# SLebailly/Ignis-MasterThesis

Measured on AMD Instinct MI355X. Metric: Mrays/s (primary+secondary) at fixed spp; per-pixel L2 vs CPU ref, higher is better.
Workload: dtype f32; 1 GPU; diamond_scene.json 1000x1000, 256 spp = 32 iterations x spi 8, path tracer max_depth 64, seed 0; scene=diamond_scene.json, width=1000, height=1000, spp=256, spi=8, parallelism=single GPU

## Files before the change

### ignis-masterthesis_amd/csrc/igx_device.hip

```cpp
#include "igx.h"

#include "device_math.h"
#include "device_scene.h"
#include "igx_kernels.h"
#include "../host/bvh_build.h"
#include "../host/light_select.h"

#include <hip/hip_runtime.h>

#include <algorithm>
#include <array>
#include <chrono>
#include <map>
#include <cmath>
#include <cstring>
#include <condition_variable>
#include <deque>
#include <memory>
#include <mutex>
#include <string>
#include <thread>
#include <vector>
#include <type_traits>

using namespace igxd;

#ifndef IGX_PART
#define IGX_PART 0
#endif

namespace igxh {

constexpr int BLOCK = 256;
[[maybe_unused]] constexpr int MAX_BLOCKS_PER_CU = 8;
[[maybe_unused]] constexpr int MAX_STACK = 128;
constexpr int MAX_BOUNCES = 256;
constexpr long long MAX_CHUNK_PATHS = 1ll << 27;
constexpr int SLOT_BITS = 27;
constexpr uint32_t SLOT_MASK = (1u << SLOT_BITS) - 1;
[[maybe_unused]] constexpr int MAX_ENCLOSING = 31;
static_assert(MAX_CHUNK_PATHS <= (1ll << SLOT_BITS), "path slots must fit the slot bits");
#ifndef EXTEND_WAVES
#define EXTEND_WAVES 4
#endif
#ifndef EXTEND_WAVES_FULL
#define EXTEND_WAVES_FULL 3
#endif
#ifndef EXTEND_WAVES_LDS
// ... 108 lines not shown
}

static_assert(NSH == 64 && BLOCK % 64 == 0 && NSH % WAVES_PER_BLOCK == 0, "one shard counter per lane of a wave");
static_assert(BLOCK == TSTACK_STRIDE, "traversal stacks are laid out for BLOCK threads");

__device__ __forceinline__ int row_total(const int* row) {
    const int* r = row + lane_id() * CSTRIDE;
    int v = r[0] + r[1] + r[2];
    for (int off = 32; off > 0; off >>= 1) v += __shfl_xor(v, off);
    return __builtin_amdgcn_readfirstlane(v);
}

struct WaveWork {
    int s, k, K;
};
__device__ __forceinline__ WaveWork wave_work() {
    const int g = __builtin_amdgcn_readfirstlane((int)blockIdx.x * WAVES_PER_BLOCK + (int)(threadIdx.x >> 6));
    return WaveWork{g % NSH, g / NSH, (int)gridDim.x * WAVES_PER_BLOCK / NSH};
}

__device__ __forceinline__ int gen_index(int i, int shard_cap) {
    return ((i >> 6) & (NSH - 1)) * shard_cap + ((i >> 12) << 6) + (i & 63);
}
__device__ __forceinline__ int gen_shard_count(int n, int s) {
    const int rem = (n & (64 * NSH - 1)) - s * 64;
    return (n >> 12) * 64 + (rem < 0 ? 0 : (rem > 64 ? 64 : rem));
}

struct ShardCount {
    int a, ab, n;
};
__device__ __forceinline__ ShardCount shard_count(const int* cnt, int s) {
    const int a = uniform_load(cnt + s * CSTRIDE), b = uniform_load(cnt + s * CSTRIDE + 1);
// ... 495 lines not shown
    const GenPath g = gen_path(fa, sv, i);
    PathState ps;
    ps.o = g.o;
    ps.d = g.d;
    ps.counter = g.counter;
    ps.seed = g.seed;
    ps.depth = g.depth;
    ps.slot = i;
    ps.contrib = mk(1, 1, 1);
    ps.inv_pdf = 0;
    ps.eta = 1.0f;
    ps.inside = -1;
    return ps;
}

template <int V0, bool STATS, bool LDS>
__global__ void __launch_bounds__(BLOCK, LDS ? EXTEND_WAVES_LDS : (variant_full(V0) ? EXTEND_WAVES_FULL : EXTEND_WAVES)) k_extend(FrameArgs fa, SceneView gsv, PathBuf in, PathBuf out, ShadowBuf sh,
                                                  float4* L, KernelCounters kc, int tail_threshold) {
    constexpr int V = LDS ? kernel_variant(V0, true) : (EXTEND_TREELET ? kernel_variant(V0, false) : V0);
    __shared__ int stack_mem[LDS_STACK * BLOCK];
    extern __shared__ float4 lds_scene[];
    const TStack ts = make_tstack(stack_mem, LDS_STACK, gsv.spill);
    const bool gen = fa.gen_n > 0;
    if (!gen && row_total(kc.cnt_in) <= tail_threshold) return;
    const SceneView sv = LDS ? stage_scene_lds<BLOCK>(gsv, lds_scene) : stage_treelet<BLOCK>(gsv, lds_scene);
    TraceStats st{0, 0, 0, 0, 0, 0, 0};
    __shared__ unsigned long long cls_mem[STATS ? WAVES_PER_BLOCK * 36 : 1];
    if constexpr (STATS) {
        st.cls = cls_mem + 36 * (threadIdx.x >> 6);
        if (lane_id() < 36) st.cls[lane_id()] = 0;
    }
    const WaveWork w = wave_work();
    int s = w.s;
    auto count_of = [&](int sh_) {
        if (gen) {
            const int g = gen_shard_count(fa.gen_n, sh_);
            return ShardCount{g, g, g};
        }
        return shard_count(kc.cnt_in, sh_);
    };
    ShardCount sc = count_of(s);
    uint64_t done = 0;
    int p0 = w.k * 64;
    int claimed = -1;
    unsigned long long t_last = STATS ? __builtin_amdgcn_s_memtime() : 0;
    for (;;) {
        if (fa.dynamic) {
// ... 724 lines not shown
    int stream_slots = 2;
    int concurrent_opt = 1;
    int concurrent_start_pct = 10;
    int tail_pairs_opt = -1;
    int64_t treelet_opt = -1;
    bool tree_dirty = true;
    int tree_ext = 0, tree_shadow = 0;
    int64_t tail_opt = -1;
    int64_t tail_last_opt = -1;
    bool fuse_generate = true;
    int split_opt = -1;
    int refill_opt = -1;
    int shadow_ifif_opt = -1;
    int64_t lds_scene_max = 48 * 1024;
    size_t lds_scene_bytes = 0;
    size_t table_bytes = 0;
    size_t shading_bytes = 0;
    int leaf_size = 4;
    int classify_opt = 4;
    int shadow_classes_opt = 1;
    int dynamic_opt = DYN_EXTEND | DYN_REFILL_TRACE | DYN_REFILL_SHADOW;
    int group_order_opt = -1;
    int face_normals_opt = 1;
    int face_shade_opt = 1;
    float sah_node_cost = 1.0f;
    int bvh_bins = 32;
    int bvh_bins_tlas = 32;
    bool spatial_splits = false;
    bool rebuild_bvh = false;
    bool has_scene = false;
// ... 146 lines not shown
    s.pa.shard_cap = s.pb.shard_cap = s.sh.shard_cap = shard_cap;
    s.cap = cap;
    s.shard_cap = shard_cap;
    return IGX_OK;
}

hipEvent_t slot_event(Slot& s) {
    if (s.ev_next >= s.ev_pool.size()) {
        hipEvent_t e;
        (void)hipEventCreate(&e);
        s.ev_pool.push_back(e);
    }
    return s.ev_pool[s.ev_next++];
}

int grid_for(igx_device* dev, long long items, int blocks_per_cu) {
    const long long q = GRID_QUANTUM;
    long long need = (items + BLOCK - 1) / BLOCK;
    long long cap = (long long)dev->num_cus * std::min(blocks_per_cu, MAX_BLOCKS_PER_CU);
    long long g = std::min((need + q - 1) / q * q, std::max(q, cap / q * q));
    return (int)std::max(q, g);
}

#endif

constexpr size_t SPLIT_TABLE_BYTES = 64u << 20;
#ifndef GROUP_ORDER_AUTO
#define GROUP_ORDER_AUTO 0
#endif
inline bool use_tail_pairs(const igx_device* dev) {
    return dev->lds_scene_bytes == 0 && (dev->tail_pairs_opt < 0 ? true : dev->tail_pairs_opt != 0);
}
inline size_t tree_bytes(const igx_device* dev, int nodes) { return (size_t)nodes * dev->nf4 * 16; }
inline int refill_min(const igx_device* dev) { return dev->refill_opt >= 0 ? dev->refill_opt : 16; }
// ... 25 lines not shown
        case 1: MACRO(1); break;              \
        case 2: MACRO(2); break;              \
        case 3: MACRO(3); break;              \
        case 4: MACRO(4); break;              \
        case 5: MACRO(5); break;              \
        case 6: MACRO(6); break;              \
        case 7: MACRO(7); break;              \
        case 2 | VARIANT_Q4: MACRO(130); break; \
        case 3 | VARIANT_Q4: MACRO(131); break; \
        case 6 | VARIANT_Q4: MACRO(134); break; \
        default: MACRO(135); break;           \
        }                                     \
    } while (0)

template <bool STATS>
void launch_extend(igx_device* dev, Slot& s, int grid, const FrameArgs& fa, const PathBuf& in, const PathBuf& out,
                   const KernelCounters& kc, int tail) {
    if (dev->lds_scene_bytes) {
#define L_EXTL(S) hipLaunchKernelGGL((k_extend<S, STATS, true>), dim3(grid), dim3(BLOCK), dev->lds_scene_bytes, dev->stream, fa, dev->sv, in, out, s.sh, s.L, kc, tail)
        IGX_DISPATCH_VARIANT8(dev->variant, L_EXTL);
#undef L_EXTL
        return;
    }
    SceneView tsv = dev->sv;
    tsv.tree_n = dev->tree_ext;
#define L_EXT(S) hipLaunchKernelGGL((k_extend<S, STATS, false>), dim3(grid), dim3(BLOCK), tree_bytes(dev, tsv.tree_n), dev->stream, fa, tsv, in, out, s.sh, s.L, kc, tail)
    IGX_DISPATCH_VARIANT8(dev->variant, L_EXT);
#undef L_EXT
}
template <bool STATS>
void launch_trace(igx_device* dev, Slot& s, int grid, const FrameArgs& fa, const PathBuf& in, const int* cnt, int tail,
                  int* work) {
// ... 62 lines not shown
#undef L_FINL
        return;
    }
    if (use_tail_pairs(dev)) {
#define L_FINP(S) hipLaunchKernelGGL((k_finish_pairs<S, STATS>), dim3(grid), dim3(BLOCK), tree_bytes(dev, tsv.tree_n), dev->tail_stream, fa, tsv, in, s.L, cnt, tail, dev->dstats, dev->tail_counts)
        IGX_DISPATCH_VARIANT8(dev->variant, L_FINP);
#undef L_FINP
        return;
    }
#define L_FIN(S) hipLaunchKernelGGL((k_finish<S, STATS, false>), dim3(grid), dim3(BLOCK), tree_bytes(dev, tsv.tree_n), dev->tail_stream, fa, tsv, in, s.L, cnt, tail, dev->dstats, dev->tail_counts)
    IGX_DISPATCH_VARIANT8(dev->variant, L_FIN);
#undef L_FIN
}

template <typename K>
int resident_blocks(K kernel, size_t dyn_lds = 0) {
    int nb = 0;
    if (hipOccupancyMaxActiveBlocksPerMultiprocessor(&nb, kernel, BLOCK, dyn_lds) != hipSuccess || nb < 1) nb = 1;
    return nb;
}
#define IGX_RES1(K, V, ...) return lds ? resident_blocks(K<V, __VA_ARGS__, true>, lds) : resident_blocks(K<V, __VA_ARGS__, false>, tree)
#define IGX_RESIDENT(K, ...)                                         \
    do {                                                             \
        switch (v & (3 | VARIANT_Q4)) {                              \
        case 0: IGX_RES1(K, 0, __VA_ARGS__);                         \
        case 1: IGX_RES1(K, 1, __VA_ARGS__);                         \
        case 2: IGX_RES1(K, 2, __VA_ARGS__);                         \
        case 3: IGX_RES1(K, 3, __VA_ARGS__);                         \
        case 2 | VARIANT_Q4: IGX_RES1(K, 130, __VA_ARGS__);          \
        default: IGX_RES1(K, 131, __VA_ARGS__);                      \
        }                                                            \
    } while (0)
#define IGX_RESIDENT8(K, ...)                                        \
    do {                                                             \
// ... 52 lines not shown
int shade_blocks_per_cu(bool full) { return full ? resident_blocks(k_shade<true>) : resident_blocks(k_shade<false>); }
#endif

#define IGX_EXTEND_HELPERS(X, S)                                                                                     \
    X void launch_extend<S>(igx_device*, Slot&, int, const FrameArgs&, const PathBuf&, const PathBuf&,               \
                            const KernelCounters&, int);                                                             \
    X int extend_blocks_per_cu<S>(int, size_t, size_t);
#define IGX_FINISH_HELPERS(X, S)                                                                                     \
    X void launch_finish<S>(igx_device*, Slot&, int, const FrameArgs&, const PathBuf&, const int*, int);             \
    X int finish_blocks_per_cu<S>(int, size_t, size_t, bool);
#define IGX_TRACE_HELPERS(X, S)                                                                                      \
    X void launch_trace<S>(igx_device*, Slot&, int, const FrameArgs&, const PathBuf&, const int*, int, int*);              \
    X void launch_shadow<S>(igx_device*, Slot&, int, const int*, int*, hipStream_t);                                       \
    X int trace_blocks_per_cu<S>(int, size_t, bool);                                                                  \
    X int shadow_blocks_per_cu<S>(int, size_t, bool, size_t);
#if IGX_PART == 1
IGX_EXTEND_HELPERS(template, true)
IGX_EXTEND_HELPERS(template, false)
#else
IGX_EXTEND_HELPERS(extern template, true)
IGX_EXTEND_HELPERS(extern template, false)
#endif
#if IGX_PART == 2
IGX_FINISH_HELPERS(template, true)
IGX_FINISH_HELPERS(template, false)
#else
IGX_FINISH_HELPERS(extern template, true)
IGX_FINISH_HELPERS(extern template, false)
#endif
#if IGX_PART == 3
// ... 43 lines not shown
    if ((st = ::wait_idle(dev)) || (st = harvest(dev, dev->slots[0])) || (st = harvest(dev, dev->slots[1]))) return st;
    HIPCHK(hipStreamSynchronize(dev->stream));
    HIPCHK(hipStreamSynchronize(dev->stream2));
    HIPCHK(hipStreamSynchronize(dev->shadow_stream));
    HIPCHK(hipStreamSynchronize(dev->tail_stream));
    unsigned long long tc[2] = {0, 0};
    HIPCHK(hipMemcpy(tc, dev->tail_counts, sizeof(tc), hipMemcpyDeviceToHost));
    HIPCHK(hipMemset(dev->tail_counts, 0, sizeof(tc)));
    dev->stats.bounce_rays += tc[0];
    dev->stats.shadow_rays += tc[1];
    dev->stats.tail_bounce_rays += tc[0];
    dev->stats.tail_shadow_rays += tc[1];
    return IGX_OK;
}

void configure_treelet(igx_device* dev) {
    dev->tree_ext = dev->tree_shadow = 0;
    dev->tree_dirty = false;
    if (!dev->has_scene || dev->lds_scene_bytes || dev->treelet_opt == 0) return;
    int cap = (int)std::min<size_t>(TREELET_FRONT, (size_t)dev->sv.num_nodes);
    if (dev->treelet_opt > 0) cap = (int)std::min<int64_t>(cap, dev->treelet_opt);
    const int v = dev->variant;
    const bool refill = use_refill(dev);
    auto fit = [&](auto blocks) {
        const int nb0 = blocks((size_t)0);
        int lo = 0, hi = cap;
        while (lo < hi) {
            const int mid = (lo + hi + 1) / 2;
            if (blocks(tree_bytes(dev, mid)) >= nb0) lo = mid;
            else hi = mid - 1;
// ... 63 lines not shown
extern "C" igx_status igx_create(int hip_device, igx_device** out) {
    if (!out) return IGX_ERR_INVALID_ARGUMENT;
    *out = nullptr;
    igx_device* dev = new igx_device();
    dev->hip_device = hip_device;
    hipError_t e = hipSetDevice(hip_device);
    if (e != hipSuccess) {
        delete dev;
        return IGX_ERR_HIP;
    }
    hipDeviceProp_t prop;
    if (hipGetDeviceProperties(&prop, hip_device) == hipSuccess) {
        dev->num_cus = prop.multiProcessorCount;
        dev->mem_total = prop.totalGlobalMem;
    }
    if (hipStreamCreateWithFlags(&dev->stream, hipStreamNonBlocking) != hipSuccess ||
        hipStreamCreateWithFlags(&dev->stream2, hipStreamNonBlocking) != hipSuccess ||
        hipStreamCreateWithFlags(&dev->tail_stream, hipStreamNonBlocking) != hipSuccess ||
        hipStreamCreateWithFlags(&dev->shadow_stream, hipStreamNonBlocking) != hipSuccess) {
        delete dev;
        return IGX_ERR_HIP;
    }
    if (hipMalloc((void**)&dev->dstats, DSTATS * sizeof(unsigned long long)) != hipSuccess ||
        hipMalloc((void**)&dev->tail_counts, 2 * sizeof(unsigned long long)) != hipSuccess) {
        delete dev;
        return IGX_ERR_OUT_OF_MEMORY;
    }
    (void)hipMemset(dev->dstats, 0, DSTATS * sizeof(unsigned long long));
    (void)hipMemset(dev->tail_counts, 0, 2 * sizeof(unsigned long long));
    *out = dev;
// ... 84 lines not shown
    else if (k == "fuse_generate") dev->fuse_generate = value != 0;
    else if (k == "split") {
        if (value < -1 || value > 1) return fail(dev, IGX_ERR_INVALID_ARGUMENT, "split must be -1 (auto), 0 or 1");
        dev->split_opt = (int)value;
    }
    else if (k == "shadow_ifif") {
        if (value < -1 || value > 1) return fail(dev, IGX_ERR_INVALID_ARGUMENT, "shadow_ifif must be -1 (auto), 0 or 1");
        dev->shadow_ifif_opt = (int)value;
    }
    else if (k == "refill") {
        if (value < -1 || value > 64) return fail(dev, IGX_ERR_INVALID_ARGUMENT, "refill must be -1 (auto) or in [0, 64]");
        dev->refill_opt = (int)value;
    }
    else if (k == "lds_scene_max") {
        dev->lds_scene_max = value;
        size_t b = ((size_t)dev->sv.num_nodes * dev->sv.node_f4 + (size_t)dev->sv.num_inst * 4 +
                    (size_t)dev->sv.num_tris * 3) * 16;
        dev->lds_scene_bytes = dev->has_scene && (int64_t)b <= value ? b : 0;
    }
    else if (k == "full_shading") dev->full_shading_opt = value != 0;
    else if (k == "enclosing") dev->enclosing_opt = value != 0;
    else if (k == "bvh_width") {
        if (value != 0 && value != 2 && value != 4) return fail(dev, IGX_ERR_INVALID_ARGUMENT, "bvh_width must be 0 (auto), 2 or 4");
        dev->bvh_width_opt = (int)value;
    }
    else if (k == "spatial_splits") dev->spatial_splits = value != 0;
    else if (k == "rebuild_bvh") dev->rebuild_bvh = value != 0;
    else if (k == "dynamic") dev->dynamic_opt = (int)(value & 15);
    else if (k == "group_order") {
        if (value < -1 || value > 1) return fail(dev, IGX_ERR_INVALID_ARGUMENT, "group_order must be -1 (auto), 0 (A, B, C) or 1 (C, B, A)");
        dev->group_order_opt = (int)value;
    }
    else if (k == "face_normals") dev->face_normals_opt = value != 0;
// ... 628 lines not shown
    }
    if (fn_tab.empty()) sv.fn_tab = nullptr;
    if (fsh.empty()) sv.fsh = nullptr;
    if (uvs.empty()) sv.uv = nullptr;
    sv.tlas_root = tlas_root;
    sv.num_nodes = (int)(nodes.size() / nf4);
    sv.node_f4 = nf4;
    dev->bvh_width = width;
    dev->quantized = quantize;
    dev->nf4 = nf4;
    sv.num_inst = (int)(inst.size() / 4);
    sv.num_enc = (int)enc_tab.size();
    sv.num_tris = (int)(tris.size() / 3);
    {
        size_t b = ((size_t)sv.num_nodes * nf4 + (size_t)sv.num_inst * 4 + (size_t)sv.num_tris * 3) * 16;
        const size_t bl = b;
        dev->lds_scene_bytes = (int64_t)bl <= dev->lds_scene_max ? bl : 0;
        dev->table_bytes = b;
        dev->shading_bytes = ent.size() * sizeof(ent[0]) + vtx.size() * sizeof(vtx[0]) + nrm.size() * sizeof(nrm[0]) +
                             idx.size() * sizeof(idx[0]) + mats.size() * sizeof(DevMaterial) + lights.size() * sizeof(lights[0]) +
                             fn_tab.size() * sizeof(fn_tab[0]) + fsh.size() * sizeof(fsh[0]);
    }
    sv.num_lights = (int)lights.size();
    sv.num_infinite = num_infinite;
    sv.selector = lsel.selector;
    float dx = desc->scene_bbox_max[0] - desc->scene_bbox_min[0];
    float dy = desc->scene_bbox_max[1] - desc->scene_bbox_min[1];
    float dz = desc->scene_bbox_max[2] - desc->scene_bbox_min[2];
    sv.scene_radius = std::sqrt(dx * dx + dy * dy + dz * dz) / 2 * 1.01f;
    if (desc->technique.max_depth > 255) {
        free_scene(dev);
        return fail(dev, IGX_ERR_UNSUPPORTED, "max_depth above 255 is not supported (8-bit path depth)");
    }
// ... 24 lines not shown
    if (textured) dev->full_shading = true;
    if (dev->aov_on) dev->full_shading = true;
    for (uint32_t e = 0; textured && e < desc->num_entities; ++e) {
        const igx_entity& en = desc->entities[e];
        if (desc->materials[en.material].texture != IGX_TEXTURE_NONE && desc->shapes[en.shape].type == IGX_SHAPE_SPHERE) {
            free_scene(dev);
            return fail(dev, IGX_ERR_UNSUPPORTED, "textured material on an analytic sphere (texture coordinates of spheres are not supported)");
        }
    }
    if ((st = configure_stack(dev)) != IGX_OK) {
        free_scene(dev);
        return st;
    }
    dev->has_scene = true;
    dev->tree_dirty = true;
    return IGX_OK;
}

struct ChunkPlan {
    FrameArgs fa{};
    DevCamera cam{};
    int iteration = 0, spi = 1, count = 1, width = 1;
    long long local_pixels = 0, chunk_pixels_max = 0;
    int iters_per_chunk = 1;
    size_t slot_cap = 0;
    int max_bounces = 1, ext_bpc = 1, sh_bpc = 1, fin_bpc = 1;
    bool pairs = false;
};
struct SchedItem {
    bool clear = false;
// ... 134 lines not shown
            r.fa.chunk_iters = std::min(pl.iters_per_chunk, pl.count - r.it0);
            r.chunk_pixels = (int)std::min<long long>(pl.chunk_pixels_max, pl.local_pixels - r.px0);
            r.fa.chunk_pixel0 = (int)r.px0;
            r.fa.chunk_pixels = r.chunk_pixels;
            r.n = (long long)r.chunk_pixels * pl.spi * r.fa.chunk_iters;
            r.live = r.n;
            const long long fin_lanes = (long long)pl.fin_bpc * dev->num_cus * BLOCK / (pl.pairs ? 2 : 1);
            const int64_t topt = r.last_of_plan && dev->tail_last_opt >= 0 ? dev->tail_last_opt : dev->tail_opt;
            r.tail = topt >= 0 ? (int)std::min<int64_t>(topt, 1 << 30) : (int)std::max<long long>(32768, std::min(r.n / 64, fin_lanes));
            S.tail = r.tail;
            S.camera = valid_pixels_in_chunk(r.fa) * pl.spi * r.fa.chunk_iters;
            S.n0 = r.n;
            S.split = false;
            S.bounce_ev.clear();
            S.launched = 0;
            r.ext_grid = grid_for(dev, r.n, pl.ext_bpc);
            r.sh_grid = grid_for(dev, r.n, pl.sh_bpc);
            r.fin_grid = grid_for(dev, std::min<long long>(r.n, r.tail) * (pl.pairs ? 2 : 1), pl.fin_bpc);
            r.fuse_gen = dev->fuse_generate && r.n > r.tail;
            use_slot(r);
            IGX_CC(hipMemsetAsync(S.ctr, 0, (size_t)(2 * pl.max_bounces + 4) * CROW * sizeof(int), dev->stream));
            if (dev->dynamic_opt)
                IGX_CC(hipMemsetAsync(S.ctr + (size_t)WORK_ROW0 * CROW, 0, (size_t)4 * pl.max_bounces * CROW * sizeof(int), dev->stream));
            if (!r.fuse_gen) {
                begin_timed(S, 2, -1, dev->stream);
                hipLaunchKernelGGL(k_generate, dim3(grid_for(dev, r.n, 8)), dim3(BLOCK), 0, dev->stream, r.fa, dev->sv, S.pa, S.L, S.ctr);
                end_timed(S, dev->stream);
                IGX_CC(hipGetLastError());
            }
            restore();
            if (r.n <= r.tail) {
// ... 19 lines not shown
                    IGX_CC(q);
                    r.live = row_total(S, 2 * (r.b - 1));
                    if (r.live <= r.tail) {
                        r.switch_b = r.b - 1;
                        r.loop_done = true;
                        break;
                    }
                }
                const int b = r.b;
                PathBuf in = (b & 1) ? S.pb : S.pa, out = (b & 1) ? S.pa : S.pb;
                KernelCounters kc{row(2 * b), row(2 * (b + 1)), row(2 * b + 1), dev->dstats, row(WORK_ROW0 + 4 * b)};
                begin_timed(S, 0, b, dev->stream);
                FrameArgs fb = r.fa;
                fb.gen_n = r.fuse_gen && b == 0 ? (int)r.n : 0;
                const long long bound = IGX_LIVE_GRID && b >= 2 ? r.live : r.n;
                const int ext_grid = IGX_LIVE_GRID ? grid_for(dev, bound, pl.ext_bpc) : r.ext_grid;
                const int sh_grid = IGX_LIVE_GRID ? grid_for(dev, bound, pl.sh_bpc) : r.sh_grid;
                if (inst) launch_extend<true>(dev, S, ext_grid, fb, in, out, kc, r.tail);
                else launch_extend<false>(dev, S, ext_grid, fb, in, out, kc, r.tail);
                end_timed(S, dev->stream);
                begin_timed(S, 1, b, dev->stream);
                int* const sh_work =
                    (dev->dynamic_opt & (use_refill(dev) ? DYN_REFILL_SHADOW : DYN_SHADOW)) ? row(WORK_ROW0 + 4 * b + 2) : nullptr;
                if (inst) launch_shadow<true>(dev, S, sh_grid, row(2 * b + 1), sh_work, dev->stream);
                else launch_shadow<false>(dev, S, sh_grid, row(2 * b + 1), sh_work, dev->stream);
                end_timed(S, dev->stream);
                IGX_CC(hipGetLastError());
                IGX_CC(hipMemcpyAsync(S.pinned + (size_t)(2 * b + 1) * CROW, row(2 * b + 1), 2 * CROW * sizeof(int),
                                      hipMemcpyDeviceToHost, dev->stream));
                hipEvent_t e = slot_event(S);
                IGX_CC(hipEventRecord(e, dev->stream));
// ... 295 lines not shown
    if (dev->slot_budget_mb > 0)
        auto_chunk_paths = std::max<long long>(1ll << 20, std::min<long long>(auto_chunk_paths, slot_budget / (dev->stream_slots * path_slot_bytes)));
    long long cap = dev->capacity_opt > 0 ? dev->capacity_opt
                                          : (count > 1 ? auto_chunk_paths : std::min<long long>({total_paths, 1ll << 24, auto_chunk_paths}));
    cap = std::min<long long>(cap, MAX_CHUNK_PATHS);
    cap = std::max<long long>(p->spi, (cap / p->spi) * p->spi);
    const long long chunk_pixels_max = std::min<long long>(cap, total_paths) / p->spi;
    const int iters_per_chunk = total_paths <= cap ? (int)std::min<long long>(count, cap / total_paths) : 1;
    const size_t slot_cap = (size_t)(chunk_pixels_max * p->spi * iters_per_chunk);

    const int max_bounces = std::min(std::max(dev->sv.max_depth, 1), MAX_BOUNCES - 1);
    const bool inst = dev->instrument;
    const int sd = dev->variant;
    const size_t ldsb = dev->lds_scene_bytes;
    if (dev->tree_dirty) configure_treelet(dev);
    const int ext_bpc = inst ? extend_blocks_per_cu<true>(sd, ldsb, tree_bytes(dev, dev->tree_ext))
                             : extend_blocks_per_cu<false>(sd, ldsb, tree_bytes(dev, dev->tree_ext));
    const bool refill = use_refill(dev);
    const int tr_bpc = inst ? trace_blocks_per_cu<true>(sd, dev->lds_scene_bytes, refill)
                            : trace_blocks_per_cu<false>(sd, dev->lds_scene_bytes, refill);
    const bool full = variant_full(sd);
    const int shade_bpc = shade_blocks_per_cu(full);
    const int sh_bpc = inst ? shadow_blocks_per_cu<true>(sd, dev->lds_scene_bytes, refill, tree_bytes(dev, dev->tree_shadow))
                            : shadow_blocks_per_cu<false>(sd, dev->lds_scene_bytes, refill, tree_bytes(dev, dev->tree_shadow));
    const bool pairs = use_tail_pairs(dev);
    const int fin_bpc = inst ? finish_blocks_per_cu<true>(sd, ldsb, 0, pairs) : finish_blocks_per_cu<false>(sd, ldsb, 0, pairs);

    if (conc) {
        auto plan = std::make_shared<ChunkPlan>();
        plan->fa = fa;
        plan->cam = cam;
        plan->iteration = p->iteration;
// ... 79 lines not shown
        const bool overlap = split && dev->overlap_shadow_opt;
        hipStream_t sh_strm = overlap ? dev->shadow_stream : dev->stream;
        hipEvent_t sh_done = nullptr;
        if (n <= tail) switch_b = 0;
        for (int b = 0; switch_b < 0 && b < max_bounces; ++b) {
            long long bound = n;
            if (b >= 2) {
                HIPCHK(hipEventSynchronize(S.bounce_ev[b - 2]));
                bound = row_total(S, 2 * (b - 1));
                if (bound <= tail) {
                    switch_b = b - 1;
                    break;
                }
            }
            if (!IGX_LIVE_GRID) bound = n;
            const int ext_grid = grid_for(dev, bound, ext_bpc), tr_grid = grid_for(dev, bound, tr_bpc);
            const int shade_grid = grid_for(dev, bound, shade_bpc), sh_grid = grid_for(dev, bound, sh_bpc);
            PathBuf in = (b & 1) ? S.pb : S.pa, out = (b & 1) ? S.pa : S.pb;
            KernelCounters kc{row(2 * b), row(2 * (b + 1)), row(2 * b + 1), dev->dstats, row(WORK_ROW0 + 4 * b)};
            if (split) {
                begin_timed(5, b, dev->stream);
                int* const tr_work = (dev->dynamic_opt & DYN_REFILL_TRACE) ? row(WORK_ROW0 + 4 * b) : nullptr;
                if (inst) launch_trace<true>(dev, S, tr_grid, fa, in, row(2 * b), tail, tr_work);
                else launch_trace<false>(dev, S, tr_grid, fa, in, row(2 * b), tail, tr_work);
                end_timed(dev->stream);
                if (sh_done) HIPCHK(hipStreamWaitEvent(dev->stream, sh_done, 0));
                begin_timed(0, b, dev->stream);
                launch_shade(dev, full, shade_grid, fa, in, S.hb, out, S.sh, S.L, kc, tail);
                end_timed(dev->stream);
            } else {
                begin_timed(0, b, dev->stream);
// ... 224 lines not shown
    out->leaf_visits = h[1];
    out->tri_tests = h[2];
    out->blas_enters = h[3];
    out->shadow_node_visits = h[4];
    out->shadow_leaf_visits = h[5];
    out->shadow_tri_tests = h[6];
    out->shadow_blas_enters = h[7];
    out->shaded_hits = h[8];
    out->wave_node_iters = h[9];
    out->wave_leaf_iters = h[10];
    out->shadow_wave_node_iters = h[11];
    out->shadow_wave_leaf_iters = h[12];
    out->bvh_width = dev->bvh_width;
    out->node_bytes = dev->nf4 * 16;
    out->lds_scene_bytes = (int32_t)dev->lds_scene_bytes;
    if (dev->has_scene && dev->tree_dirty) configure_treelet(dev);
    out->shadow_blocks_per_cu = dev->has_scene ? shadow_blocks_per_cu<false>(dev->variant, dev->lds_scene_bytes, use_refill(dev),
                                                                            tree_bytes(dev, dev->tree_shadow)) : 0;
    out->treelet_nodes[0] = dev->tree_ext;
    out->treelet_nodes[1] = 0;
    out->treelet_nodes[2] = dev->tree_shadow;
    out->treelet_nodes[3] = 0;
    out->table_bytes = dev->table_bytes;
    out->shading_bytes = dev->shading_bytes;
    out->slot_bytes = 0;
    for (const Slot& s : dev->slots)
        out->slot_bytes += (uint64_t)s.shard_cap * NSH * (2 * 56 * (s.pa.c_base ? 2 : 1) + 48 + (s.hb.h ? 20 : 0)) +
                           (uint64_t)s.cap * (16 + (s.aov_di ? 32 : 0));
    return IGX_OK;
}
// ... 62 lines not shown
```

### ignis-masterthesis_amd/csrc/igx_kernels.h

```cpp
#pragma once

#include "device_math.h"
#include "device_scene.h"

namespace igxd {

struct SceneView {
    const float4* nodes;
    const float4* tris;
    const float4* inst;
    const float4* spheres;
    const float4* ent;
    const float4* vtx;
    const float4* nrm;
    const int4* idx;
    const DevMaterial* mats;
    const DevLight* lights;
    int tlas_root;
    int num_lights;
    int num_infinite;
    float scene_radius;
    DevCamera cam;
    int max_depth, min_depth, nee;
    float clamp;
// ... 1 lines not shown
    const float4* tree;
    int tree_n;
    int* spill;
    int node_f4;
    const int* ent_enc;
    const int2* enc;
    const float4* enc_box;
    int num_enc;
    int selector;
    const float* sel_cdf;
    const uint32_t* sel_tree;
    const int* ent_fn;
    const float4* fn_tab;
    const float4* fsh;
    const float2* uv;
};

constexpr int MAX_ENC_BOXES = 32;
template <int BLOCK_>
__device__ __forceinline__ const float4* stage_enc_boxes(const SceneView& sv) {
    __shared__ float4 enc_box_lds[2 * MAX_ENC_BOXES];
    for (int k = threadIdx.x; k < 2 * sv.num_enc; k += BLOCK_) enc_box_lds[k] = sv.enc_box[k];
    return enc_box_lds;
}

template <int BLOCK_>
__device__ __forceinline__ SceneView stage_scene_lds(const SceneView& sv, float4* lds) {
    const int nf = sv.node_f4, sh = nf == 8 ? 3 : 2, ns = nf;
    const int n4 = sv.num_nodes * ns, i4 = sv.num_inst * 4, t3 = sv.num_tris * 3;
    for (int k = threadIdx.x; k < sv.num_nodes * nf; k += BLOCK_) lds[(k >> sh) * ns + (k & (nf - 1))] = sv.nodes[k];
    for (int k = threadIdx.x; k < i4; k += BLOCK_) lds[n4 + k] = sv.inst[k];
    for (int k = threadIdx.x; k < t3; k += BLOCK_) lds[n4 + i4 + k] = sv.tris[k];
    const float4* eb = stage_enc_boxes<BLOCK_>(sv);
    __syncthreads();
    SceneView l = sv;
    l.enc_box = eb;
    l.nodes = lds;
    l.inst = lds + n4;
    l.tris = lds + n4 + i4;
    return l;
}

template <int BLOCK_>
__device__ __forceinline__ SceneView stage_treelet(const SceneView& sv, float4* lds) {
    SceneView l = sv;
    l.tree = lds;
    if (sv.tree_n > 0 || sv.num_enc > 0) {
        const int n4 = sv.tree_n * sv.node_f4;
        for (int k = threadIdx.x; k < n4; k += BLOCK_) lds[k] = sv.nodes[k];
        l.enc_box = stage_enc_boxes<BLOCK_>(sv);
// ... 122 lines not shown
        const int top = sp + n - 2;
        if (top + 1 < s.cap) {
            const int dead = top + 1;
            lds_int* col = (lds_int*)s.lds;
            col[top * TSTACK_STRIDE] = r1;
            col[(n > 2 ? top - 1 : dead) * TSTACK_STRIDE] = r2;
            col[(n > 3 ? top - 2 : dead) * TSTACK_STRIDE] = r3;
            sp = top + 1;
            return;
        }
    }
    if (n > 3) tpush<SPILL>(s, sp, r3);
    if (n > 2) tpush<SPILL>(s, sp, r2);
    if (n > 1) tpush<SPILL>(s, sp, r1);
}
__device__ __forceinline__ TStack make_tstack(int* lds_base, int cap, int* spill) {
    const int g = blockIdx.x * TSTACK_STRIDE + threadIdx.x;
    return TStack{lds_base + threadIdx.x, spill + g, cap, (int)(gridDim.x * TSTACK_STRIDE)};
}

__device__ __forceinline__ bool accept_hit(const Trav& t, float th, int ent, int prim) {
    return th >= t.tmin && (th < t.tmax || (th == t.tmax && (ent > t.hit_ent || (ent == t.hit_ent && prim > t.hit_prim))));
}

__device__ __forceinline__ void trav_init(const SceneView& sv, Trav& t, f3 o, f3 d, float tmin, float tmax, uint32_t rflags,
                                          const TStack& ts) {
    t.o = o;
    t.d = d;
    t.lo = o;
    t.ld = d;
    t.idir = mk(safe_rcp(d.x), safe_rcp(d.y), safe_rcp(d.z));
    t.iorg = mk(-(o.x * t.idir.x), -(o.y * t.idir.y), -(o.z * t.idir.z));
    t.tmin = tmin;
// ... 1549 lines not shown
```

### ignis-masterthesis_amd/ignis_amd/_native.py

```python
import ctypes as C
import os

_PKG_DIR = os.path.dirname(os.path.abspath(__file__))
LIB_PATH = os.environ.get("IGX_LIB_PATH") or os.path.join(os.path.dirname(_PKG_DIR), "libigx.so")



class Mesh(C.Structure):
    _fields_ = [("num_vertices", C.c_uint32), ("num_faces", C.c_uint32),
                ("vertices", C.POINTER(C.c_float)), ("normals", C.POINTER(C.c_float)),
                ("texcoords", C.POINTER(C.c_float)), ("indices", C.POINTER(C.c_uint32))]


class Shape(C.Structure):
    _fields_ = [("type", C.c_int32), ("mesh", C.c_int32), ("sphere", C.c_float * 4),
                ("bbox_min", C.c_float * 3), ("bbox_max", C.c_float * 3), ("is_plane", C.c_int32),
                ("plane_origin", C.c_float * 3), ("plane_x", C.c_float * 3), ("plane_y", C.c_float * 3),
                ("plane_tex", C.c_float * 8), ("ref_bvh", C.c_void_p), ("ref_bvh_bytes", C.c_uint64)]


class Entity(C.Structure):
    _fields_ = [("shape", C.c_int32), ("material", C.c_int32), ("flags", C.c_uint32),
                ("to_global", C.c_float * 12), ("to_local", C.c_float * 12), ("normal", C.c_float * 9),
                ("bbox_min", C.c_float * 3), ("bbox_max", C.c_float * 3)]
# ... 86 lines not shown
                ("launches_trace", C.c_uint64), ("ms_trace", C.c_double),
                ("wave_node_iters", C.c_uint64), ("wave_leaf_iters", C.c_uint64),
                ("shadow_wave_node_iters", C.c_uint64), ("shadow_wave_leaf_iters", C.c_uint64),
                ("bvh_width", C.c_int32), ("node_bytes", C.c_int32),
                ("lds_scene_bytes", C.c_int32), ("shadow_blocks_per_cu", C.c_int32),
                ("table_bytes", C.c_uint64), ("shading_bytes", C.c_uint64),
                ("extend_cycles_load", C.c_uint64), ("extend_cycles_trace", C.c_uint64),
                ("extend_cycles_shade", C.c_uint64), ("extend_cycles_store", C.c_uint64),
                ("slot_bytes", C.c_uint64), ("treelet_nodes", C.c_int32 * 4),
                ("extend_class_cycles", C.c_uint64 * 8), ("extend_class_groups", C.c_uint64 * 4),
                ("extend_class_node_iters", C.c_uint64 * 4), ("extend_class_node_visits", C.c_uint64 * 4),
                ("shadow_class_groups", C.c_uint64 * 2), ("shadow_class_node_iters", C.c_uint64 * 2),
                ("shadow_class_node_visits", C.c_uint64 * 2), ("shadow_class_cycles", C.c_uint64 * 2),
                ("shadow_class_occluded", C.c_uint64 * 2), ("tlas_node_visits", C.c_uint64),
                ("hot_node_visits", C.c_uint64 * 3), ("extend_class_shade_cycles", C.c_uint64 * 16),
                ("shadow_class_rays", C.c_uint64 * 2)]

    def as_dict(self):
        return {name: (list(getattr(self, name)) if isinstance(getattr(self, name), C.Array) else getattr(self, name))
                for name, _ in self._fields_}


EXPORTED_SYMBOLS = [
    "igx_scene_load_file", "igx_scene_load_string", "igx_scene_get_desc", "igx_scene_free", "igx_write_exr",
    "igx_scene_from_database", "igx_scene_find_material", "igx_scene_entity_name",
    "igx_create", "igx_destroy", "igx_last_error", "igx_version", "igx_set_option", "igx_upload_scene",
    "igx_render", "igx_get_framebuffer", "igx_framebuffer_device_ptr", "igx_get_aov", "igx_aov_device_ptr",
    "igx_pack_tiles", "igx_clear", "igx_get_stats", "igx_reset_stats", "igx_trace_hits", "igx_trace_occlusion", "igx_synchronize", "igx_wait_ready",
    "igx_render_iterations", "igx_objscene_create", "igx_objscene_free", "igx_objscene_add",
    "igx_objscene_set_property", "igx_scene_from_objects", "igx_set_camera",
]
# ... 70 lines not shown
```

### include/igx.h

```cpp
#ifndef IGX_H
#define IGX_H

#include <stddef.h>
#include <stdint.h>

#include "igx_scene.h"

#ifdef __cplusplus
extern "C" {
#endif

typedef enum igx_status {
    IGX_OK = 0,
    IGX_ERR_INVALID_ARGUMENT = 1,
    IGX_ERR_HIP = 2,
    IGX_ERR_OUT_OF_MEMORY = 3,
    IGX_ERR_NO_SCENE = 4,
    IGX_ERR_UNSUPPORTED = 5
} igx_status;

typedef struct igx_device igx_device;

typedef struct igx_render_params {
    int32_t width, height;
// ... 40 lines not shown
    int32_t shadow_blocks_per_cu;
    uint64_t table_bytes;
    uint64_t shading_bytes;
    uint64_t extend_cycles_load, extend_cycles_trace, extend_cycles_shade, extend_cycles_store;
    uint64_t slot_bytes;
    int32_t treelet_nodes[4];
    uint64_t extend_class_cycles[8];
    uint64_t extend_class_groups[4];
    uint64_t extend_class_node_iters[4];
    uint64_t extend_class_node_visits[4];
    uint64_t shadow_class_groups[2], shadow_class_node_iters[2], shadow_class_node_visits[2];
    uint64_t shadow_class_cycles[2], shadow_class_occluded[2];
    uint64_t tlas_node_visits, hot_node_visits[3];
    uint64_t extend_class_shade_cycles[16];
    uint64_t shadow_class_rays[2];
} igx_stats;

igx_status igx_create(int hip_device, igx_device** out);
igx_status igx_destroy(igx_device* dev);
const char* igx_last_error(const igx_device* dev);
const char* igx_version(void);

igx_status igx_set_option(igx_device* dev, const char* key, int64_t value);

igx_status igx_upload_scene(igx_device* dev, const igx_scene_desc* desc);

igx_status igx_set_camera(igx_device* dev, const igx_camera* camera);

igx_status igx_render(igx_device* dev, const igx_render_params* params);
igx_status igx_render_iterations(igx_device* dev, const igx_render_params* params, int32_t count);
// ... 23 lines not shown
```

Before: 13630 Mrays/s.

## Stage shading tables in LDS with a 1024-thread extend kernel variant

```diff
diff --git a/ignis-masterthesis_amd/csrc/igx_device.hip b/ignis-masterthesis_amd/csrc/igx_device.hip
--- a/ignis-masterthesis_amd/csrc/igx_device.hip
+++ b/ignis-masterthesis_amd/csrc/igx_device.hip
@@ -5,6 +5,7 @@
 #include "igx_kernels.h"
 #include "../host/bvh_build.h"
 #include "../host/light_select.h"
+#include "../host/lds_plan.h"
 
 #include <hip/hip_runtime.h>
 
@@ -32,6 +33,8 @@
 namespace igxh {
 
 constexpr int BLOCK = 256;
+constexpr int BLOCK_WIDE = LDS_PLAN_BLOCK_WIDE;
+static_assert(BLOCK == LDS_PLAN_BLOCK, "host/lds_plan.h plans for BLOCK-thread blocks");
 [[maybe_unused]] constexpr int MAX_BLOCKS_PER_CU = 8;
 [[maybe_unused]] constexpr int MAX_STACK = 128;
 constexpr int MAX_BOUNCES = 256;
@@ -170,9 +173,12 @@
 struct WaveWork {
     int s, k, K;
 };
+template <int BT = BLOCK>
 __device__ __forceinline__ WaveWork wave_work() {
-    const int g = __builtin_amdgcn_readfirstlane((int)blockIdx.x * WAVES_PER_BLOCK + (int)(threadIdx.x >> 6));
-    return WaveWork{g % NSH, g / NSH, (int)gridDim.x * WAVES_PER_BLOCK / NSH};
+    constexpr int WPB = BT / 64;
+    static_assert(BT % 64 == 0 && NSH % WPB == 0, "a block's waves divide the shards");
+    const int g = __builtin_amdgcn_readfirstlane((int)blockIdx.x * WPB + (int)(threadIdx.x >> 6));
+    return WaveWork{g % NSH, g / NSH, (int)gridDim.x * WPB / NSH};
 }
 
 __device__ __forceinline__ int gen_index(int i, int shard_cap) {
@@ -698,23 +704,25 @@
     return ps;
 }
 
-template <int V0, bool STATS, bool LDS>
-__global__ void __launch_bounds__(BLOCK, LDS ? EXTEND_WAVES_LDS : (variant_full(V0) ? EXTEND_WAVES_FULL : EXTEND_WAVES)) k_extend(FrameArgs fa, SceneView gsv, PathBuf in, PathBuf out, ShadowBuf sh,
+template <int V0, bool STATS, bool LDS, int BT = BLOCK>
+__global__ void __launch_bounds__(BT, LDS ? EXTEND_WAVES_LDS : (variant_full(V0) ? EXTEND_WAVES_FULL : EXTEND_WAVES)) k_extend(FrameArgs fa, SceneView gsv, PathBuf in, PathBuf out, ShadowBuf sh,
                                                   float4* L, KernelCounters kc, int tail_threshold) {
+    static_assert(BT == BLOCK || (LDS && BT == BLOCK_WIDE), "the wide block is the LDS-staged kernel's");
+    constexpr bool SHADE_LDS = BT > BLOCK;
     constexpr int V = LDS ? kernel_variant(V0, true) : (EXTEND_TREELET ? kernel_variant(V0, false) : V0);
-    __shared__ int stack_mem[LDS_STACK * BLOCK];
+    __shared__ int stack_mem[LDS_STACK * BT];
     extern __shared__ float4 lds_scene[];
-    const TStack ts = make_tstack(stack_mem, LDS_STACK, gsv.spill);
+    const TStack ts = make_tstack<BT>(stack_mem, LDS_STACK, gsv.spill);
     const bool gen = fa.gen_n > 0;
     if (!gen && row_total(kc.cnt_in) <= tail_threshold) return;
-    const SceneView sv = LDS ? stage_scene_lds<BLOCK>(gsv, lds_scene) : stage_treelet<BLOCK>(gsv, lds_scene);
+    const SceneView sv = LDS ? stage_scene_lds<BT, SHADE_LDS>(gsv, lds_scene) : stage_treelet<BT>(gsv, lds_scene);
     TraceStats st{0, 0, 0, 0, 0, 0, 0};
-    __shared__ unsigned long long cls_mem[STATS ? WAVES_PER_BLOCK * 36 : 1];
+    __shared__ unsigned long long cls_mem[STATS ? BT / 64 * 36 : 1];
     if constexpr (STATS) {
         st.cls = cls_mem + 36 * (threadIdx.x >> 6);
         if (lane_id() < 36) st.cls[lane_id()] = 0;
     }
-    const WaveWork w = wave_work();
+    const WaveWork w = wave_work<BT>();
     int s = w.s;
     auto count_of = [&](int sh_) {
         if (gen) {
@@ -1469,6 +1477,12 @@
     int shadow_ifif_opt = -1;
     int64_t lds_scene_max = 48 * 1024;
     size_t lds_scene_bytes = 0;
+    int lds_shading_opt = -1;
+    int64_t lds_shading_max = 48 * 1024;
+    size_t lds_shading_bytes = 0;
+    int ext_block = BLOCK;
+    size_t lds_shading_tab[LDS_TAB_COUNT] = {};
+    size_t lds_per_block = 64 * 1024;
     size_t table_bytes = 0;
     size_t shading_bytes = 0;
     int leaf_size = 4;
@@ -1645,10 +1659,10 @@
     return s.ev_pool[s.ev_next++];
 }
 
-int grid_for(igx_device* dev, long long items, int blocks_per_cu) {
-    const long long q = GRID_QUANTUM;
-    long long need = (items + BLOCK - 1) / BLOCK;
-    long long cap = (long long)dev->num_cus * std::min(blocks_per_cu, MAX_BLOCKS_PER_CU);
+int grid_for(igx_device* dev, long long items, int blocks_per_cu, int block = BLOCK) {
+    const long long q = NSH / (block / 64);
+    long long need = (items + block - 1) / block;
+    long long cap = (long long)dev->num_cus * std::min(blocks_per_cu, MAX_BLOCKS_PER_CU * BLOCK / block);
     long long g = std::min((need + q - 1) / q * q, std::max(q, cap / q * q));
     return (int)std::max(q, g);
 }
@@ -1704,8 +1718,40 @@
     } while (0)
 
 template <bool STATS>
+void launch_extend_wide(igx_device* dev, Slot& s, int grid, const FrameArgs& fa, const PathBuf& in, const PathBuf& out,
+                        const KernelCounters& kc, int tail) {
+    const size_t dyn = lds_pad16(dev->lds_scene_bytes) + dev->lds_shading_bytes;
+#define L_EXTW(S) hipLaunchKernelGGL((k_extend<S, STATS, true, BLOCK_WIDE>), dim3(grid), dim3(BLOCK_WIDE), dyn, dev->stream, fa, dev->sv, in, out, s.sh, s.L, kc, tail)
+    IGX_DISPATCH_VARIANT8(dev->variant, L_EXTW);
+#undef L_EXTW
+}
+template <typename K>
+hipError_t raise_dynamic_lds(K kernel, size_t dyn) {
+    static std::map<std::pair<const void*, int>, size_t> raised;
+    int d = 0;
+    (void)hipGetDevice(&d);
+    const void* const fn = reinterpret_cast<const void*>(kernel);
+    size_t& have = raised[{fn, d}];
+    if (dyn <= have) return hipSuccess;
+    const hipError_t e = hipFuncSetAttribute(fn, hipFuncAttributeMaxDynamicSharedMemorySize, (int)dyn);
+    if (e == hipSuccess) have = dyn;
+    return e;
+}
+template <bool STATS>
+hipError_t extend_wide_prepare(int v, size_t dyn) {
+#define L_PREP(S) return raise_dynamic_lds(k_extend<S, STATS, true, BLOCK_WIDE>, dyn)
+    IGX_DISPATCH_VARIANT8(v, L_PREP);
+#undef L_PREP
+    return hipSuccess;
+}
+
+template <bool STATS>
 void launch_extend(igx_device* dev, Slot& s, int grid, const FrameArgs& fa, const PathBuf& in, const PathBuf& out,
                    const KernelCounters& kc, int tail) {
+    if (dev->ext_block == BLOCK_WIDE) {
+        launch_extend_wide<STATS>(dev, s, grid, fa, in, out, kc, tail);
+        return;
+    }
     if (dev->lds_scene_bytes) {
 #define L_EXTL(S) hipLaunchKernelGGL((k_extend<S, STATS, true>), dim3(grid), dim3(BLOCK), dev->lds_scene_bytes, dev->stream, fa, dev->sv, in, out, s.sh, s.L, kc, tail)
         IGX_DISPATCH_VARIANT8(dev->variant, L_EXTL);
@@ -1798,10 +1844,17 @@
 }
 
 template <typename K>
-int resident_blocks(K kernel, size_t dyn_lds = 0) {
+int resident_blocks(K kernel, size_t dyn_lds = 0, int block = BLOCK) {
     int nb = 0;
-    if (hipOccupancyMaxActiveBlocksPerMultiprocessor(&nb, kernel, BLOCK, dyn_lds) != hipSuccess || nb < 1) nb = 1;
+    if (hipOccupancyMaxActiveBlocksPerMultiprocessor(&nb, kernel, block, dyn_lds) != hipSuccess || nb < 1) nb = 1;
     return nb;
+}
+template <bool STATS>
+int extend_wide_blocks_per_cu(int v, size_t dyn) {
+#define L_RW(S) return resident_blocks(k_extend<S, STATS, true, BLOCK_WIDE>, dyn, BLOCK_WIDE)
+    IGX_DISPATCH_VARIANT8(v, L_RW);
+#undef L_RW
+    return 1;
 }
 #define IGX_RES1(K, V, ...) return lds ? resident_blocks(K<V, __VA_ARGS__, true>, lds) : resident_blocks(K<V, __VA_ARGS__, false>, tree)
 #define IGX_RESIDENT(K, ...)                                         \
@@ -1884,6 +1937,18 @@
     X void launch_shadow<S>(igx_device*, Slot&, int, const int*, int*, hipStream_t);                                       \
     X int trace_blocks_per_cu<S>(int, size_t, bool);                                                                  \
     X int shadow_blocks_per_cu<S>(int, size_t, bool, size_t);
+#define IGX_EXTEND_WIDE_HELPERS(X, S)                                                                                \
+    X void launch_extend_wide<S>(igx_device*, Slot&, int, const FrameArgs&, const PathBuf&, const PathBuf&,          \
+                                 const KernelCounters&, int);                                                        \
+    X hipError_t extend_wide_prepare<S>(int, size_t);                                                                \
+    X int extend_wide_blocks_per_cu<S>(int, size_t);
+#if IGX_PART == 4
+IGX_EXTEND_WIDE_HELPERS(template, true)
+IGX_EXTEND_WIDE_HELPERS(template, false)
+#else
+IGX_EXTEND_WIDE_HELPERS(extern template, true)
+IGX_EXTEND_WIDE_HELPERS(extern template, false)
+#endif
 #if IGX_PART == 1
 IGX_EXTEND_HELPERS(template, true)
 IGX_EXTEND_HELPERS(template, false)
@@ -1957,6 +2022,42 @@
     return IGX_OK;
 }
 
+#ifndef LDS_SHADING_AUTO
+#define LDS_SHADING_AUTO 1
+#endif
+constexpr size_t EXTEND_FIXED_LDS = 2 * MAX_ENC_BOXES * sizeof(float4) + BLOCK_WIDE / 64 * 36 * sizeof(unsigned long long);
+void configure_lds(igx_device* dev) {
+    dev->lds_scene_bytes = dev->lds_shading_bytes = 0;
+    dev->ext_block = BLOCK;
+    if (!dev->has_scene) return;
+    LdsPlanInput in;
+    in.traversal_bytes = dev->table_bytes;
+    in.traversal_max = dev->lds_scene_max;
+    for (int k = 0; k < LDS_TAB_COUNT; ++k) in.shading_bytes[k] = dev->lds_shading_tab[k];
+    in.shading_max = dev->lds_shading_max;
+    in.shading_on = dev->lds_shading_opt < 0 ? LDS_SHADING_AUTO != 0 : dev->lds_shading_opt != 0;
+    in.stack_bytes_per_thread = LDS_STACK * sizeof(int);
+    in.fixed_bytes = EXTEND_FIXED_LDS;
+    in.lds_per_block = dev->lds_per_block;
+    LdsPlan p = plan_lds(in);
+    if (p.block_threads == BLOCK_WIDE) {
+        const size_t dyn = lds_pad16(p.traversal_bytes) + p.shading_bytes;
+        (void)hipSetDevice(dev->hip_device);
+        hipError_t e = extend_wide_prepare<false>(dev->variant, dyn);
+        if (e == hipSuccess) e = extend_wide_prepare<true>(dev->variant, dyn);
+        if (e != hipSuccess) {
+            (void)hipGetLastError();
+            dev->last_error = std::string("lds_shading: the wide k_extend's LDS block was refused (") + hipGetErrorString(e) +
+                              "); keeping the 256-thread layout";
+            p.block_threads = BLOCK;
+            p.shading_bytes = 0;
+        }
+    }
+    dev->lds_scene_bytes = p.traversal_bytes;
+    dev->lds_shading_bytes = p.shading_bytes;
+    dev->ext_block = p.block_threads;
+}
+
 void configure_treelet(igx_device* dev) {
     dev->tree_ext = dev->tree_shadow = 0;
     dev->tree_dirty = false;
@@ -2050,6 +2151,9 @@
         dev->num_cus = prop.multiProcessorCount;
         dev->mem_total = prop.totalGlobalMem;
     }
+    int lds_block = 0;
+    if (hipDeviceGetAttribute(&lds_block, hipDeviceAttributeMaxSharedMemoryPerBlock, hip_device) == hipSuccess && lds_block > 0)
+        dev->lds_per_block = (size_t)lds_block;
     if (hipStreamCreateWithFlags(&dev->stream, hipStreamNonBlocking) != hipSuccess ||
         hipStreamCreateWithFlags(&dev->stream2, hipStreamNonBlocking) != hipSuccess ||
         hipStreamCreateWithFlags(&dev->tail_stream, hipStreamNonBlocking) != hipSuccess ||
@@ -2164,9 +2268,16 @@
     }
     else if (k == "lds_scene_max") {
         dev->lds_scene_max = value;
-        size_t b = ((size_t)dev->sv.num_nodes * dev->sv.node_f4 + (size_t)dev->sv.num_inst * 4 +
-                    (size_t)dev->sv.num_tris * 3) * 16;
-        dev->lds_scene_bytes = dev->has_scene && (int64_t)b <= value ? b : 0;
+        configure_lds(dev);
+    }
+    else if (k == "lds_shading") {
+        if (value < -1 || value > 1) return fail(dev, IGX_ERR_INVALID_ARGUMENT, "lds_shading must be -1 (auto), 0 or 1");
+        dev->lds_shading_opt = (int)value;
+        configure_lds(dev);
+    }
+    else if (k == "lds_shading_max") {
+        dev->lds_shading_max = value;
+        configure_lds(dev);
     }
     else if (k == "full_shading") dev->full_shading_opt = value != 0;
     else if (k == "enclosing") dev->enclosing_opt = value != 0;
@@ -2825,9 +2936,17 @@
     sv.num_tris = (int)(tris.size() / 3);
     {
         size_t b = ((size_t)sv.num_nodes * nf4 + (size_t)sv.num_inst * 4 + (size_t)sv.num_tris * 3) * 16;
-        const size_t bl = b;
-        dev->lds_scene_bytes = (int64_t)bl <= dev->lds_scene_max ? bl : 0;
         dev->table_bytes = b;
+        sv.num_ent = (int)(ent.size() / ENT_STRIDE);
+        sv.num_fsh = (int)(fsh.size() / 3);
+        sv.num_fn = (int)fn_tab.size();
+        sv.num_mats = (int)mats.size();
+        dev->lds_shading_tab[LDS_TAB_ENT] = ent.size() * sizeof(ent[0]);
+        dev->lds_shading_tab[LDS_TAB_FSH] = fsh.size() * sizeof(fsh[0]);
+        dev->lds_shading_tab[LDS_TAB_FN] = fn_tab.size() * sizeof(fn_tab[0]);
+        dev->lds_shading_tab[LDS_TAB_MATS] = mats.size() * sizeof(DevMaterial);
+        dev->lds_shading_tab[LDS_TAB_LIGHTS] = lights.size() * sizeof(lights[0]);
+        dev->lds_shading_tab[LDS_TAB_ENT_ENC] = ent_enc.size() * sizeof(ent_enc[0]);
         dev->shading_bytes = ent.size() * sizeof(ent[0]) + vtx.size() * sizeof(vtx[0]) + nrm.size() * sizeof(nrm[0]) +
                              idx.size() * sizeof(idx[0]) + mats.size() * sizeof(DevMaterial) + lights.size() * sizeof(lights[0]) +
                              fn_tab.size() * sizeof(fn_tab[0]) + fsh.size() * sizeof(fsh[0]);
@@ -2882,6 +3001,7 @@
     }
     dev->has_scene = true;
     dev->tree_dirty = true;
+    configure_lds(dev);
     return IGX_OK;
 }
 
@@ -3046,7 +3166,7 @@
             S.split = false;
             S.bounce_ev.clear();
             S.launched = 0;
-            r.ext_grid = grid_for(dev, r.n, pl.ext_bpc);
+            r.ext_grid = grid_for(dev, r.n, pl.ext_bpc, dev->ext_block);
             r.sh_grid = grid_for(dev, r.n, pl.sh_bpc);
             r.fin_grid = grid_for(dev, std::min<long long>(r.n, r.tail) * (pl.pairs ? 2 : 1), pl.fin_bpc);
             r.fuse_gen = dev->fuse_generate && r.n > r.tail;
@@ -3096,7 +3216,7 @@
                 FrameArgs fb = r.fa;
                 fb.gen_n = r.fuse_gen && b == 0 ? (int)r.n : 0;
                 const long long bound = IGX_LIVE_GRID && b >= 2 ? r.live : r.n;
-                const int ext_grid = IGX_LIVE_GRID ? grid_for(dev, bound, pl.ext_bpc) : r.ext_grid;
+                const int ext_grid = IGX_LIVE_GRID ? grid_for(dev, bound, pl.ext_bpc, dev->ext_block) : r.ext_grid;
                 const int sh_grid = IGX_LIVE_GRID ? grid_for(dev, bound, pl.sh_bpc) : r.sh_grid;
                 if (inst) launch_extend<true>(dev, S, ext_grid, fb, in, out, kc, r.tail);
                 else launch_extend<false>(dev, S, ext_grid, fb, in, out, kc, r.tail);
@@ -3422,8 +3542,11 @@
     const int sd = dev->variant;
     const size_t ldsb = dev->lds_scene_bytes;
     if (dev->tree_dirty) configure_treelet(dev);
-    const int ext_bpc = inst ? extend_blocks_per_cu<true>(sd, ldsb, tree_bytes(dev, dev->tree_ext))
-                             : extend_blocks_per_cu<false>(sd, ldsb, tree_bytes(dev, dev->tree_ext));
+    const size_t wide_dyn = lds_pad16(ldsb) + dev->lds_shading_bytes;
+    const int ext_bpc = dev->ext_block == BLOCK_WIDE
+                            ? (inst ? extend_wide_blocks_per_cu<true>(sd, wide_dyn) : extend_wide_blocks_per_cu<false>(sd, wide_dyn))
+                            : (inst ? extend_blocks_per_cu<true>(sd, ldsb, tree_bytes(dev, dev->tree_ext))
+                                    : extend_blocks_per_cu<false>(sd, ldsb, tree_bytes(dev, dev->tree_ext)));
     const bool refill = use_refill(dev);
     const int tr_bpc = inst ? trace_blocks_per_cu<true>(sd, dev->lds_scene_bytes, refill)
                             : trace_blocks_per_cu<false>(sd, dev->lds_scene_bytes, refill);
@@ -3533,7 +3656,7 @@
                 }
             }
             if (!IGX_LIVE_GRID) bound = n;
-            const int ext_grid = grid_for(dev, bound, ext_bpc), tr_grid = grid_for(dev, bound, tr_bpc);
+            const int ext_grid = grid_for(dev, bound, ext_bpc, dev->ext_block), tr_grid = grid_for(dev, bound, tr_bpc);
             const int shade_grid = grid_for(dev, bound, shade_bpc), sh_grid = grid_for(dev, bound, sh_bpc);
             PathBuf in = (b & 1) ? S.pb : S.pa, out = (b & 1) ? S.pa : S.pb;
             KernelCounters kc{row(2 * b), row(2 * (b + 1)), row(2 * b + 1), dev->dstats, row(WORK_ROW0 + 4 * b)};
@@ -3788,6 +3911,8 @@
     out->bvh_width = dev->bvh_width;
     out->node_bytes = dev->nf4 * 16;
     out->lds_scene_bytes = (int32_t)dev->lds_scene_bytes;
+    out->lds_shading_bytes = (int32_t)dev->lds_shading_bytes;
+    out->extend_block_threads = dev->ext_block;
     if (dev->has_scene && dev->tree_dirty) configure_treelet(dev);
     out->shadow_blocks_per_cu = dev->has_scene ? shadow_blocks_per_cu<false>(dev->variant, dev->lds_scene_bytes, use_refill(dev),
                                                                             tree_bytes(dev, dev->tree_shadow)) : 0;
diff --git a/ignis-masterthesis_amd/csrc/igx_kernels.h b/ignis-masterthesis_amd/csrc/igx_kernels.h
--- a/ignis-masterthesis_amd/csrc/igx_kernels.h
+++ b/ignis-masterthesis_amd/csrc/igx_kernels.h
@@ -39,6 +39,7 @@
     const float4* fn_tab;
     const float4* fsh;
     const float2* uv;
+    int num_ent, num_fsh, num_fn, num_mats;
 };
 
 constexpr int MAX_ENC_BOXES = 32;
@@ -49,7 +50,7 @@
     return enc_box_lds;
 }
 
-template <int BLOCK_>
+template <int BLOCK_, bool SHADE = false>
 __device__ __forceinline__ SceneView stage_scene_lds(const SceneView& sv, float4* lds) {
     const int nf = sv.node_f4, sh = nf == 8 ? 3 : 2, ns = nf;
     const int n4 = sv.num_nodes * ns, i4 = sv.num_inst * 4, t3 = sv.num_tris * 3;
@@ -57,8 +58,31 @@
     for (int k = threadIdx.x; k < i4; k += BLOCK_) lds[n4 + k] = sv.inst[k];
     for (int k = threadIdx.x; k < t3; k += BLOCK_) lds[n4 + i4 + k] = sv.tris[k];
     const float4* eb = stage_enc_boxes<BLOCK_>(sv);
+    SceneView l = sv;
+    if constexpr (SHADE) {
+        constexpr int M4 = sizeof(DevMaterial) / 16, L4 = sizeof(DevLight) / 16;
+        float4* const s_ent = lds + n4 + i4 + t3;
+        float4* const s_fsh = s_ent + sv.num_ent * ENT_STRIDE;
+        float4* const s_fn = s_fsh + sv.num_fsh * 3;
+        float4* const s_mats = s_fn + sv.num_fn;
+        float4* const s_lights = s_mats + sv.num_mats * M4;
+        int* const s_enc = reinterpret_cast<int*>(s_lights + sv.num_lights * L4);
+        const float4* const g_mats = reinterpret_cast<const float4*>(sv.mats);
+        const float4* const g_lights = reinterpret_cast<const float4*>(sv.lights);
+        for (int k = threadIdx.x; k < sv.num_ent * ENT_STRIDE; k += BLOCK_) s_ent[k] = sv.ent[k];
+        for (int k = threadIdx.x; k < sv.num_fsh * 3; k += BLOCK_) s_fsh[k] = sv.fsh[k];
+        for (int k = threadIdx.x; k < sv.num_fn; k += BLOCK_) s_fn[k] = sv.fn_tab[k];
+        for (int k = threadIdx.x; k < sv.num_mats * M4; k += BLOCK_) s_mats[k] = g_mats[k];
+        for (int k = threadIdx.x; k < sv.num_lights * L4; k += BLOCK_) s_lights[k] = g_lights[k];
+        for (int k = threadIdx.x; k < sv.num_ent; k += BLOCK_) s_enc[k] = sv.ent_enc[k];
+        l.ent = s_ent;
+        l.fsh = s_fsh;
+        l.fn_tab = s_fn;
+        l.mats = reinterpret_cast<const DevMaterial*>(s_mats);
+        l.lights = reinterpret_cast<const DevLight*>(s_lights);
+        l.ent_enc = s_enc;
+    }
     __syncthreads();
-    SceneView l = sv;
     l.enc_box = eb;
     l.nodes = lds;
     l.inst = lds + n4;
@@ -211,9 +235,13 @@
     if (n > 2) tpush<SPILL>(s, sp, r2);
     if (n > 1) tpush<SPILL>(s, sp, r1);
 }
+template <int BT = TSTACK_STRIDE>
 __device__ __forceinline__ TStack make_tstack(int* lds_base, int cap, int* spill) {
-    const int g = blockIdx.x * TSTACK_STRIDE + threadIdx.x;
-    return TStack{lds_base + threadIdx.x, spill + g, cap, (int)(gridDim.x * TSTACK_STRIDE)};
+    static_assert(BT % TSTACK_STRIDE == 0, "a block is a whole number of stack regions");
+    const int g = blockIdx.x * BT + threadIdx.x;
+    int* col = lds_base + threadIdx.x;
+    if constexpr (BT > TSTACK_STRIDE) col = lds_base + (threadIdx.x / TSTACK_STRIDE) * (LDS_STACK * TSTACK_STRIDE) + threadIdx.x % TSTACK_STRIDE;
+    return TStack{col, spill + g, cap, (int)(gridDim.x * BT)};
 }
 
 __device__ __forceinline__ bool accept_hit(const Trav& t, float th, int ent, int prim) {
diff --git a/ignis-masterthesis_amd/host/lds_plan.h b/ignis-masterthesis_amd/host/lds_plan.h
--- /dev/null
+++ b/ignis-masterthesis_amd/host/lds_plan.h
@@ -0,0 +1,51 @@
+#pragma once
+
+#include <stddef.h>
+#include <stdint.h>
+
+namespace igxh {
+
+constexpr int LDS_PLAN_BLOCK = 256;
+constexpr int LDS_PLAN_BLOCK_WIDE = 1024;
+enum { LDS_TAB_ENT = 0, LDS_TAB_FSH, LDS_TAB_FN, LDS_TAB_MATS, LDS_TAB_LIGHTS, LDS_TAB_ENT_ENC, LDS_TAB_COUNT };
+
+struct LdsPlanInput {
+    size_t traversal_bytes = 0;
+    int64_t traversal_max = 0;
+    size_t shading_bytes[LDS_TAB_COUNT] = {};
+    int64_t shading_max = 0;
+    bool shading_on = false;
+    size_t stack_bytes_per_thread = 0;
+    size_t fixed_bytes = 0;
+    size_t lds_per_block = 0;
+};
+
+struct LdsPlan {
+    int block_threads = LDS_PLAN_BLOCK;
+    size_t traversal_bytes = 0;
+    size_t shading_bytes = 0;
+};
+
+constexpr size_t lds_pad16(size_t b) { return (b + 15) & ~(size_t)15; }
+
+inline size_t lds_shading_total(const LdsPlanInput& in) {
+    size_t t = 0;
+    for (int k = 0; k < LDS_TAB_COUNT; ++k) t += lds_pad16(in.shading_bytes[k]);
+    return t;
+}
+
+inline LdsPlan plan_lds(const LdsPlanInput& in) {
+    LdsPlan p;
+    if (in.traversal_max <= 0 || in.traversal_bytes == 0 || (int64_t)in.traversal_bytes > in.traversal_max) return p;
+    p.traversal_bytes = in.traversal_bytes;
+    if (!in.shading_on || in.shading_bytes[LDS_TAB_FSH] == 0 || in.shading_bytes[LDS_TAB_FN] == 0) return p;
+    const size_t sh = lds_shading_total(in);
+    if ((int64_t)sh > in.shading_max) return p;
+    const size_t block = (size_t)LDS_PLAN_BLOCK_WIDE * in.stack_bytes_per_thread + in.fixed_bytes + lds_pad16(in.traversal_bytes) + sh;
+    if (block > in.lds_per_block) return p;
+    p.block_threads = LDS_PLAN_BLOCK_WIDE;
+    p.shading_bytes = sh;
+    return p;
+}
+
+}
diff --git a/ignis-masterthesis_amd/ignis_amd/_native.py b/ignis-masterthesis_amd/ignis_amd/_native.py
--- a/ignis-masterthesis_amd/ignis_amd/_native.py
+++ b/ignis-masterthesis_amd/ignis_amd/_native.py
@@ -124,7 +124,8 @@
                 ("shadow_class_node_visits", C.c_uint64 * 2), ("shadow_class_cycles", C.c_uint64 * 2),
                 ("shadow_class_occluded", C.c_uint64 * 2), ("tlas_node_visits", C.c_uint64),
                 ("hot_node_visits", C.c_uint64 * 3), ("extend_class_shade_cycles", C.c_uint64 * 16),
-                ("shadow_class_rays", C.c_uint64 * 2)]
+                ("shadow_class_rays", C.c_uint64 * 2),
+                ("lds_shading_bytes", C.c_int32), ("extend_block_threads", C.c_int32)]
 
     def as_dict(self):
         return {name: (list(getattr(self, name)) if isinstance(getattr(self, name), C.Array) else getattr(self, name))
diff --git a/include/igx.h b/include/igx.h
--- a/include/igx.h
+++ b/include/igx.h
@@ -78,6 +78,8 @@
     uint64_t tlas_node_visits, hot_node_visits[3];
     uint64_t extend_class_shade_cycles[16];
     uint64_t shadow_class_rays[2];
+    int32_t lds_shading_bytes;
+    int32_t extend_block_threads;
 } igx_stats;
 
 igx_status igx_create(int hip_device, igx_device** out);
```

Result: faster. 14160 Mrays/s, median of 6 (+3.9%).
